# smoggy-P/gym-Drone2D-ActivePerception

Measured on AMD Instinct MI355X. Metric: env-steps/sec (batched) at 10 agents, map_id=1, higher is better.
Workload: dtype f64

## Files before the change

gym-drone2d-activeperception_amd/csrc/d2d_plugins.h:

```cpp

#define D2D_SINCOS_QUAL __device__ __forceinline__
#define D2D_SINCOS_TBL_QUAL __device__ const
#include "d2d_sincos.h"
#define D2D_ATAN2_QUAL __device__ __forceinline__
#define D2D_ATAN2_TBL_QUAL __device__ const
#include "d2d_atan2.h"
#define D2D_POW2_QUAL __device__ __forceinline__
#define D2D_POW2_TBL_QUAL __device__ const
#include "d2d_pow2.h"

__device__ __forceinline__ double norm2(double x, double y) { return sqrt(__builtin_fma(y, y, x * x)); }

__device__ __forceinline__ double shfl_f64(double v, int src) {
  int lo = __double2loint(v), hi = __double2hiint(v);
  lo = __shfl(lo, src, WAVE);
  hi = __shfl(hi, src, WAVE);
  return __hiloint2double(hi, lo);
}

template <int N>
__device__ __forceinline__ double row_shl_f64(double v) {
  int lo = __double2loint(v), hi = __double2hiint(v);
  lo = __builtin_amdgcn_update_dpp(lo, lo, 0x100 + N, 0xf, 0xf, false);
  hi = __builtin_amdgcn_update_dpp(hi, hi, 0x100 + N, 0xf, 0xf, false);
  return __hiloint2double(hi, lo);
}

template <int N>
__device__ __forceinline__ int row_shr_i32(int v) { return __builtin_amdgcn_update_dpp(v, v, 0x110 + N, 0xf, 0xf, false); }
template <int N>
__device__ __forceinline__ double row_shr_f64(double v) {
  return __hiloint2double(row_shr_i32<N>(__double2hiint(v)), row_shr_i32<N>(__double2loint(v)));
}
__device__ __forceinline__ double readlane_f64(double v, int l) {
  return __hiloint2double(__builtin_amdgcn_readlane(__double2hiint(v), l), __builtin_amdgcn_readlane(__double2loint(v), l));
}

__device__ __forceinline__ int wave_argmin(double t, int idx) {
  double m = t;
  m = __builtin_fmin(m, row_shr_f64<1>(m));
  m = __builtin_fmin(m, row_shr_f64<2>(m));
  m = __builtin_fmin(m, row_shr_f64<4>(m));
  m = __builtin_fmin(m, row_shr_f64<8>(m));
  const double wmin = __builtin_fmin(__builtin_fmin(readlane_f64(m, 15), readlane_f64(m, 31)),
                                     __builtin_fmin(readlane_f64(m, 47), readlane_f64(m, 63)));
  const unsigned long long eq = __ballot(t == wmin);
  if (__popcll(eq) == 1) return __builtin_amdgcn_readlane(idx, __ffsll((long long)eq) - 1);
  int c = (t == wmin) ? idx : 0x7fffffff;
  c = min(c, row_shr_i32<1>(c));
  c = min(c, row_shr_i32<2>(c));
  c = min(c, row_shr_i32<4>(c));
  c = min(c, row_shr_i32<8>(c));
  return min(min(__builtin_amdgcn_readlane(c, 15), __builtin_amdgcn_readlane(c, 31)),
             min(__builtin_amdgcn_readlane(c, 47), __builtin_amdgcn_readlane(c, 63)));
}

__device__ __forceinline__ double wave_fmin(double m) {
  m = __builtin_fmin(m, row_shr_f64<1>(m));
  m = __builtin_fmin(m, row_shr_f64<2>(m));
  m = __builtin_fmin(m, row_shr_f64<4>(m));
  m = __builtin_fmin(m, row_shr_f64<8>(m));
  return __builtin_fmin(__builtin_fmin(readlane_f64(m, 15), readlane_f64(m, 31)), __builtin_fmin(readlane_f64(m, 47), readlane_f64(m, 63)));
}
__device__ __forceinline__ double wave_fmax(double m) {
  m = __builtin_fmax(m, row_shr_f64<1>(m));
  m = __builtin_fmax(m, row_shr_f64<2>(m));
  m = __builtin_fmax(m, row_shr_f64<4>(m));
  m = __builtin_fmax(m, row_shr_f64<8>(m));
  return __builtin_fmax(__builtin_fmax(readlane_f64(m, 15), readlane_f64(m, 31)), __builtin_fmax(readlane_f64(m, 47), readlane_f64(m, 63)));
}

struct TrkView {
  double *mx, *my, *vx, *vy;
  double *lim;
  int n;
};

__device__ __forceinline__ double sq_threshold(double L) {
  if (!(L >= 0.0)) return -1.0;
  double t = L * L;
  for (int k = 0; k < 8 && sqrt(t) > L; ++k) t = __longlong_as_double(__double_as_longlong(t) - 1);
  for (int k = 0; k < 8; ++k) {
    const double u = __longlong_as_double(__double_as_longlong(t) + 1);
    if (!(sqrt(u) <= L)) break;
    t = u;
  }
  return t;
}

template <int WIDTH>
__device__ __forceinline__ bool plan_hits_round(const TrkView &T, int q, double x, double y, double t) {
  double mx[WIDTH], my[WIDTH], vx[WIDTH], vy[WIDTH], lim[WIDTH];
#pragma unroll
  for (int u = 0; u < WIDTH; ++u) {
    mx[u] = T.mx[q + u]; my[u] = T.my[q + u]; vx[u] = T.vx[q + u]; vy[u] = T.vy[q + u]; lim[u] = T.lim[q + u];
  }
  bool hit = false;
#pragma unroll
  for (int u = 0; u < WIDTH; ++u) {
    const double ex = mx[u] + t * vx[u], ey = my[u] + t * vy[u];
    const double dx = x - ex, dy = y - ey;
    hit = hit | ((q + u < T.n) & (__builtin_fma(dy, dy, dx * dx) <= lim[u]));
  }
  return hit;
}

__device__ __forceinline__ bool plan_hits_tracker(const TrkView &T, double x, double y, double t) {
  if (T.n <= 2) return T.n > 0 ? plan_hits_round<2>(T, 0, x, y, t) : false;
  bool hit = false;
  for (int q = 0; q < T.n; q += 4) hit = hit | plan_hits_round<4>(T, q, x, y, t);
  return hit;
}

template <typename DM>
__device__ __forceinline__ bool plan_is_free(const d2d_cfg &c, const d2d_plan &p, DM dm,
                                             const TrkView &T, double x, double y, double t, double inv_scale) {
  if (x != x || y != y) return false;
  const double d = p.safe_dist;
  const double xl = x - d, xr = x + d, yl = y - d, yr = y + d;
  const int W1 = c.W - 1, H1 = c.H - 1;
  const int i0 = min(max(cell_fast(xl, c.scale, inv_scale), 0), W1), i1 = min(max(cell_fast(x, c.scale, inv_scale), 0), W1),
            i2 = min(max(cell_fast(xr, c.scale, inv_scale), 0), W1);
  const int j0 = min(max(cell_fast(yl, c.scale, inv_scale), 0), H1), j1 = min(max(cell_fast(y, c.scale, inv_scale), 0), H1),
            j2 = min(max(cell_fast(yr, c.scale, inv_scale), 0), H1);
  const unsigned char v0 = dm[grid_ix(c, i0, j1)], v1 = dm[grid_ix(c, i1, j1)], v2 = dm[grid_ix(c, i2, j1)], v3 = dm[grid_ix(c, i1, j0)],
                      v4 = dm[grid_ix(c, i1, j2)];
  const bool ox0 = (xl >= c.W_px) | (xl < 0.0), ox1 = (x >= c.W_px) | (x < 0.0), ox2 = (xr >= c.W_px) | (xr < 0.0);
  const bool oy0 = (yl >= c.H_px) | (yl < 0.0), oy1 = (y >= c.H_px) | (y < 0.0), oy2 = (yr >= c.H_px) | (yr < 0.0);
  const bool wall = (ox0 | oy1 | (v0 == D2D_OCCUPIED)) | (ox1 | oy1 | (v1 == D2D_OCCUPIED)) | (ox2 | oy1 | (v2 == D2D_OCCUPIED)) |
                    (ox1 | oy0 | (v3 == D2D_OCCUPIED)) | (ox1 | oy2 | (v4 == D2D_OCCUPIED));
  return !wall && !plan_hits_tracker(T, x, y, t);
}

template <typename DM>
__device__ __forceinline__ bool plan_wall_int(const d2d_cfg &c, DM dm, int xi, int yi, int di, int Wpx, int Hpx) {
  const int xl = xi - di, xr = xi + di, yl = yi - di, yr = yi + di;
  const bool ox0 = (unsigned int)xl >= (unsigned int)Wpx, ox1 = (unsigned int)xi >= (unsigned int)Wpx, ox2 = (unsigned int)xr >= (unsigned int)Wpx;
  const bool oy0 = (unsigned int)yl >= (unsigned int)Hpx, oy1 = (unsigned int)yi >= (unsigned int)Hpx, oy2 = (unsigned int)yr >= (unsigned int)Hpx;
  const int Wm = Wpx - 1, Hm = Hpx - 1;
#define D2D_BY10(v, m) ((int)(__umul24((unsigned int)min(max((v), 0), (m)), 52429u) >> 19))
  const int W1 = c.W - 1, H1 = c.H - 1;
  const int i0 = min(D2D_BY10(xl, Wm), W1), i1 = min(D2D_BY10(xi, Wm), W1), i2 = min(D2D_BY10(xr, Wm), W1);
  const int j0 = min(D2D_BY10(yl, Hm), H1), j1 = min(D2D_BY10(yi, Hm), H1), j2 = min(D2D_BY10(yr, Hm), H1);
#undef D2D_BY10
  const unsigned char v0 = dm[grid_ix(c, i0, j1)], v1 = dm[grid_ix(c, i1, j1)], v2 = dm[grid_ix(c, i2, j1)], v3 = dm[grid_ix(c, i1, j0)],
                      v4 = dm[grid_ix(c, i1, j2)];
  return (ox0 | oy1 | (v0 == D2D_OCCUPIED)) | (ox1 | oy1 | (v1 == D2D_OCCUPIED)) | (ox2 | oy1 | (v2 == D2D_OCCUPIED)) |
         (ox1 | oy0 | (v3 == D2D_OCCUPIED)) | (ox1 | oy2 | (v4 == D2D_OCCUPIED));
}


__device__ __forceinline__ long long node_key(double px, double py, double vx, double vy) {
  const int a = cell_fast(rint(px), 10.0, 0.1), b = cell_fast(rint(py), 10.0, 0.1);
  const int cc = (int)rint(vx), d = (int)rint(vy);
  const unsigned int hi = ((unsigned int)(a + 32768) << 16) | ((unsigned int)(b + 32768) & 0xffffu);
  const unsigned int lo = ((unsigned int)(cc + 32768) << 16) | ((unsigned int)(d + 32768) & 0xffffu);
  return (long long)(((unsigned long long)hi << 32) | lo);
}

__device__ __forceinline__ unsigned int key_hash(long long k) {
  return (unsigned int)(((unsigned long long)k * 0x9E3779B97F4A7C15ull) >> 32);
}

#define NR_POS 0
#define NR_VEL 2
#define NR_COST 4
#define NR_META 6
#define NR_ACC 8
struct NodeRecs {
  double *b;
  __device__ __forceinline__ double *rec(int i) const { return b + (size_t)i * D2D_NODE_F; }
};
__device__ __forceinline__ double2 ld2(const double *q) { return *(const double2 *)q; }
__device__ __forceinline__ void st2(double *q, double a, double b) { *(double2 *)q = make_double2(a, b); }
__device__ __forceinline__ double meta_pack(int parent, int itr, int state) { return __hiloint2double((itr << 2) | state, parent); }
__device__ __forceinline__ int meta_parent(double m) { return __double2loint(m); }
__device__ __forceinline__ int meta_itr(double m) { return __double2hiint(m) >> 2; }
__device__ __forceinline__ int meta_state(double m) { return __double2hiint(m) & 3; }

#ifndef D2D_TRAJ_PRUNE_CHUNKS
#define D2D_TRAJ_PRUNE_CHUNKS 4
#endif
__device__ __forceinline__ double *traj_boxes(const d2d_plan &p, int e) {
  return p.traj_box ? (double *)p.traj_box + (size_t)e * ((p.traj_cap + WAVE - 1) / WAVE) * 4 : nullptr;
}

#define LH_N 1024
#define LH_MAX 896

#ifdef D2D_SEARCH_PROF
__device__ unsigned long long d2d_search_prof[16];
#define SP_T(var)                                              \
  do {                                                         \
    asm volatile("s_waitcnt vmcnt(0) lgkmcnt(0)" ::: "memory"); \
    var = __builtin_amdgcn_s_memtime();                        \
  } while (0)
#define SP_ADD(idx, t0, t1) \
  do {                      \
    spacc[idx] += (t1) - (t0); \
  } while (0)
#define SP_FLUSH()                                                            \
  do {                                                                        \
    if (e == 0 && lane == 0)                                                  \
      for (int spi = 0; spi < 16; ++spi) d2d_search_prof[spi] += spacc[spi]; \
  } while (0)
#else
#define SP_T(var) do { } while (0)
#define SP_ADD(idx, t0, t1) do { } while (0)
#define SP_FLUSH() do { } while (0)
#endif

struct SearchLds {
  int *chain;
  double *us;
  double *st;
  double *pc;
  double *rv;
  long long *rk;
  int *ri;
  int *misc;
  double *tot;
  int ntot;
  unsigned long long *prow;
  unsigned short *lh;
};

__host__ __device__ inline int search_lds_nodes(int N) { return N > 64 ? 256 : 512; }
__host__ __device__ inline bool search_wall_rows(int W, int H) { return W <= 64 && H <= 64; }

__device__ int plan_search(const d2d_cfg &c, const d2d_state &s, const d2d_plan &p, int e, int lane, const TrkView &T,
                           const SearchLds &S, const unsigned char *__restrict__ dm, double inv_scale) {
  const double H = p.horizon;
  const NodeRecs nd = {p.nodes + (size_t)e * p.node_cap * D2D_NODE_F};
  int *__restrict__ tab = p.hash + (size_t)e * p.hash_cap;
  double *__restrict__ traj = p.traj + (size_t)e * p.traj_cap * 4;
  int *stat = p.plan_stat + (size_t)e * 4;
  int *chain = S.chain;
  const unsigned int hmask = (unsigned int)p.hash_cap - 1u;
  const double tx = s.target[(size_t)e * 2], ty = s.target[(size_t)e * 2 + 1];
  const double *dr = s.drone + (size_t)e * D2D_DF;

  unsigned long long spa = 0, spb = 0;
  (void)spa; (void)spb;
#ifdef D2D_SEARCH_PROF
  unsigned long long spacc[16] = {0, 0, 0, 0, 0, 0, 0, 0, 0, 0, 0, 0, 0, 0, 0, 0};
#endif
  SP_T(spa);
  for (int i = lane; i < p.nu; i += WAVE) S.us[i] = p.u_space[i];
  {
    const FastDiv fdu(p.nu);
    for (int i = lane; i < p.nu * p.nu; i += WAVE) {
      int ia, ja;
      fdu.divmod(i, ia, ja);
      const double ax = p.u_space[ia], ay = p.u_space[ja];
      S.pc[i] = (ax * ax + ay * ay) / 100;
    }
  }
  for (int i = lane; i < 2 * p.n_sample; i += WAVE) S.st[i] = p.sample_t[i];
  {
    uint4 *lh128 = (uint4 *)S.lh;
    for (int i = lane; i < LH_N / 8; i += WAVE) lh128[i] = make_uint4(0u, 0u, 0u, 0u);
  }
  const bool int_walls = c.scale == 10.0 && c.W_px <= 81919.0 && c.H_px <= 81919.0 && c.W_px == floor(c.W_px) &&
                         c.H_px == floor(c.H_px) && c.W_px >= 1.0 && c.H_px >= 1.0 && p.safe_dist >= 0.0 &&
                         p.safe_dist <= 1048576.0 && p.safe_dist == floor(p.safe_dist);
  const int safe_i = int_walls ? (int)p.safe_dist : 0, wpx_i = int_walls ? (int)c.W_px : 1, hpx_i = int_walls ? (int)c.H_px : 1;
  const int kcell = safe_i / 10;
  const bool rows = S.prow != nullptr && int_walls && c.W <= 64 && c.H <= 64 && c.W_px == 10.0 * (double)c.W &&
                    c.H_px == 10.0 * (double)c.H && safe_i == 10 * kcell && 2 * kcell <= min(c.W, c.H);
  if (rows) {
    int olo = 0, ohi = 0;
    unsigned long long *orow = (unsigned long long *)S.rk;
    const int nb = c.W * c.H;
    if (c.grid_tile == 0 && (nb & 3) == 0 && (((size_t)dm) & 3) == 0) {
      orow[lane] = 0ull;
      const unsigned int *src = (const unsigned int *)dm;
      const FastDiv fdh(c.H);
      for (int d0 = 0; d0 < nb / 4; d0 += 10 * WAVE) {
        unsigned int x[10];
#pragma unroll
        for (int u = 0; u < 10; ++u) {
          const int idx = d0 + u * WAVE + lane;
          x[u] = src[min(idx, nb / 4 - 1)];
        }
#pragma unroll
        for (int u = 0; u < 10; ++u) {
          const int idx = d0 + u * WAVE + lane;
          const unsigned int y = x[u] ^ 0x01010101u;
          unsigned int z = ~(((y & 0x7f7f7f7fu) + 0x7f7f7f7fu) | y | 0x7f7f7f7fu);
          if (idx >= nb / 4) z = 0u;
          while (z) {
            const int b = (__ffs((int)z) - 1) >> 3;
            z &= z - 1u;
            int i, j;
            fdh.divmod_big(4 * idx + b, i, j);
            atomicOr(&orow[i], 1ull << j);
          }
        }
      }
      wave_sync_lds();
      const unsigned long long o = orow[lane];
      olo = (int)(unsigned int)o;
      ohi = (int)(unsigned int)(o >> 32);
      wave_sync_lds();
    } else {
      const int jc = min(lane, c.H - 1);
      for (int i0 = 0; i0 < c.W; i0 += 8) {
        unsigned char v[8];
#pragma unroll
        for (int u = 0; u < 8; ++u) v[u] = dm[grid_ix(c, min(i0 + u, c.W - 1), jc)];
#pragma unroll
        for (int u = 0; u < 8; ++u) {
          if (i0 + u < c.W) {
            const unsigned long long m = __ballot(lane < c.H && v[u] == D2D_OCCUPIED);
            olo = lane == i0 + u ? (int)(unsigned int)m : olo;
            ohi = lane == i0 + u ? (int)(unsigned int)(m >> 32) : ohi;
          }
        }
      }
    }
    const unsigned long long occ = ((unsigned long long)(unsigned int)ohi << 32) | (unsigned int)olo;
    orow[lane] = occ;
    wave_sync_lds();
    const unsigned long long up = orow[max(lane - kcell, 0)], dn = orow[min(lane + kcell, WAVE - 1)];
    const unsigned long long edge = kcell > 0 ? ((1ull << kcell) - 1ull) : 0ull;
    const unsigned long long edge_hi = kcell > 0 ? (edge << (c.H - kcell)) : 0ull;
    unsigned long long pr = occ | up | dn | (occ << kcell) | (occ >> kcell) | edge | edge_hi;
    if (lane < kcell || lane >= c.W - kcell) pr = ~0ull;
    wave_sync_lds();
    S.prow[lane] = pr;
  }
  const double kInf = __longlong_as_double(0x7ff0000000000000ll);
  const double vmax2 = p.vmax_sq != 0.0 ? p.vmax_sq : (p.vmax > 0.0 ? sq_threshold(__longlong_as_double(__double_as_longlong(p.vmax) - 1)) : -1.0);
  const double goal2 = p.goal_sq != 0.0 ? p.goal_sq : sq_threshold(p.goal_tol);
  wave_sync_lds();
  if (lane == 0) {
    const double x = dr[D2D_D_X], y = dr[D2D_D_Y], vx = dr[D2D_D_VX], vy = dr[D2D_D_VY];
    const double tot0 = 0.0 + 0.5 * norm2(x - tx, y - ty) + 0.1 * norm2(vx, vy);
    const long long k = node_key(x, y, vx, vy);
    double *r0 = nd.rec(0);
    st2(r0 + NR_POS, x, y);
    st2(r0 + NR_VEL, vx, vy);
    st2(r0 + NR_COST, 0.0, __longlong_as_double(k));
    st2(r0 + NR_META, meta_pack(-1, 0, 1), tot0);
    st2(r0 + NR_ACC, 0.0, 0.0);
    const unsigned int h32 = key_hash(k);
    S.lh[h32 >> 22] = (unsigned short)((((h32 >> 17) & 0x1fu) << 11) | 1u);
    S.tot[0] = tot0;
  }
  wave_sync_global();
  SP_T(spb);
  SP_ADD(10, spa, spb);
  bool nodup;
  double amax = 0.0;
  {
    double dmin = 1e300;
    for (int i = lane; i < p.nu; i += WAVE) {
      const double ui = S.us[i];
      if (i + 1 < p.nu) dmin = fmin(dmin, S.us[i + 1] - ui);
      amax = fmax(amax, fabs(ui));
    }
    dmin = wave_fmin(dmin);
    amax = wave_fmax(amax);
    nodup = H * dmin > 1.0 + 1e-6;
  }
  int nn = 1, open_n = 1, goal = -1, itr = 0, expansions = 0;
  bool overflow = false;
  bool lds_dict = true;
  const int nprim = p.nu * p.nu;
  const unsigned long long lt_mask = (1ull << lane) - 1ull;
  const FastDiv fd_nu(p.nu), fd_ns(p.n_sample);
  const double reach_a = 0.5 * H * H * amax + 2.0;
  const bool ns_pow2 = (p.n_sample & (p.n_sample - 1)) == 0 && p.n_sample <= WAVE;
  const bool one_batch = false;
  double ax1 = 0.0, ay1 = 0.0;
  if (one_batch) {
    int ia, ja;
    fd_nu.divmod(lane < nprim ? lane : 0, ia, ja);
    ax1 = S.us[ia];
    ay1 = S.us[ja];
  }
  for (;;) {
    itr += 1;
    if (open_n == 0 || itr >= p.max_itr) break;
    unsigned long long sp0 = 0, sp1 = 0, sp2 = 0, sp3 = 0, sp4 = 0, sp5 = 0, sp6 = 0, sp7 = 0, sp8 = 0;
    (void)sp0; (void)sp1; (void)sp2; (void)sp3; (void)sp4; (void)sp5; (void)sp6; (void)sp7; (void)sp8;
    SP_T(sp0);
    double best = kInf;
    int bidx = 0x7fffffff;
    bool fenced = false;
    {
      const int nl = min(nn, S.ntot);
      for (int s0 = 0; s0 < nl; s0 += 4 * WAVE) {
        double t4[4];
#pragma unroll
        for (int u = 0; u < 4; ++u) t4[u] = S.tot[min(s0 + u * WAVE + lane, S.ntot - 1)];
#pragma unroll
        for (int u = 0; u < 4; ++u) {
          const int si = s0 + u * WAVE + lane;
          const bool take = (si < nl) & (t4[u] < best);
          best = take ? t4[u] : best;
          bidx = take ? si : bidx;
        }
      }
      if (nn > nl) {
        wave_sync_global();
        fenced = true;
      }
      for (int s0 = nl; s0 < nn; s0 += WAVE) {
        const int si = s0 + lane;
        const double2 mt = ld2(nd.rec(min(si, nn - 1)) + NR_META);
        const bool take = (si < nn) & (meta_state(mt.x) == 1) & (mt.y < best);
        best = take ? mt.y : best;
        bidx = take ? si : bidx;
      }
    }
    bidx = wave_argmin(best, bidx);
    if (!fenced) wave_sync_global();
    if (__builtin_amdgcn_readfirstlane(bidx) == 0x7fffffff) {
      int fb = 0x7fffffff;
      for (int s0 = 0; s0 < nn; s0 += WAVE) {
        const int si = s0 + lane;
        if (si < nn && fb == 0x7fffffff && meta_state(nd.rec(si)[NR_META]) == 1) fb = si;
      }
      for (int o = 32; o > 0; o >>= 1) fb = min(fb, __shfl_xor(fb, o, WAVE));
      bidx = fb;
    }
    const int cur = __builtin_amdgcn_readfirstlane(bidx);
    SP_T(sp1);
    SP_ADD(0, sp0, sp1);
    const double *rc = nd.rec(cur);
    const double2 cpos = ld2(rc + NR_POS), cvel = ld2(rc + NR_VEL);
    const double ccost = rc[NR_COST];
    const int citr = meta_itr(rc[NR_META]);
    const double px = cpos.x, py = cpos.y, vx = cvel.x, vy = cvel.y;
    const bool fits_all = int_walls && (fabs(px) + H * fabs(vx) + reach_a <= 4194304.0) && (fabs(py) + H * fabs(vy) + reach_a <= 4194304.0);
    SP_T(sp2);
    SP_ADD(1, sp1, sp2);
    if (__builtin_fma(py - ty, py - ty, (px - tx) * (px - tx)) <= goal2) {
      goal = cur;
      break;
    }
    if (lane == 0) {
      ((int *)(nd.rec(cur) + NR_META))[1] = (citr << 2) | 2;
      if (cur < S.ntot) S.tot[cur] = kInf;
    }
    open_n -= 1;
    expansions += 1;
    for (int p0 = 0; p0 < nprim && !overflow; p0 += WAVE) {
      const int pi = p0 + lane;
      bool ok = pi < nprim;
      double ax, ay;
      if (one_batch) {
        ax = ax1;
        ay = ay1;
      } else {
        int ia, ja;
        fd_nu.divmod(ok ? pi : 0, ia, ja);
        ax = S.us[ia];
        ay = S.us[ja];
      }
      const double hx = ax / 2, hy = ay / 2;
      const double vex = vx + (2 * H) * hx, vey = vy + (2 * H) * hy;
      ok = ok && (__builtin_fma(vey, vey, vex * vex) <= vmax2);
      const unsigned long long vm = __ballot(ok);
      const int myrank = __popcll(vm & lt_mask);
      SP_T(sp3);
      SP_ADD(2, sp2, sp3);
      {
        const int nv = __popcll(vm);
        double *rax = S.rv, *ray = (double *)S.rk;
        if (ok) {
          rax[myrank] = hx;
          ray[myrank] = hy;
        }
        wave_sync_lds();
        const int npair = nv * p.n_sample;
        const int my_lo = myrank * p.n_sample;
        int nfree = 0;
        for (int q0 = 0; q0 < npair; q0 += 2 * WAVE) {
          int pr[2], si[2];
          bool in[2], fr[2];
          double sxv[2], syv[2], tgv[2];
#pragma unroll
          for (int u = 0; u < 2; ++u) {
            const int q = q0 + u * WAVE + lane;
            in[u] = q < npair;
            fd_ns.divmod(in[u] ? q : 0, pr[u], si[u]);
          }
          double shx[2], shy[2], tt[2], tt2[2];
#pragma unroll
          for (int u = 0; u < 2; ++u) {
            shx[u] = rax[pr[u]]; shy[u] = ray[pr[u]]; tt[u] = S.st[2 * si[u]]; tt2[u] = S.st[2 * si[u] + 1];
          }
#pragma unroll
          for (int u = 0; u < 2; ++u) {
            const double sx = rint(__builtin_fma(tt2[u], shx[u], px + tt[u] * vx)), sy = rint(__builtin_fma(tt2[u], shy[u], py + tt[u] * vy));
            const double tg = tt[u] + (double)citr * H;
            sxv[u] = sx; syv[u] = sy; tgv[u] = tg;
          }
          if (fits_all) {
            bool wall[2];
#pragma unroll
            for (int u = 0; u < 2; ++u) {
              const int xi = (int)sxv[u], yi = (int)syv[u];
              if (rows) {
                const bool inside = ((unsigned int)xi < (unsigned int)wpx_i) & ((unsigned int)yi < (unsigned int)hpx_i);
                unsigned int ci = __umul24((unsigned int)xi, 52429u) >> 19;
                ci = ci < 63u ? ci : 63u;
                const unsigned int cj = (__umul24((unsigned int)yi, 52429u) >> 19) & 63u;
                wall[u] = !inside | (((S.prow[ci] >> cj) & 1ull) != 0ull);
              } else {
                wall[u] = plan_wall_int(c, dm, xi, yi, safe_i, wpx_i, hpx_i);
              }
            }
#pragma unroll
            for (int u = 0; u < 2; ++u) fr[u] = !wall[u] & !plan_hits_tracker(T, sxv[u], syv[u], tgv[u]);
          } else {
#pragma unroll
            for (int u = 0; u < 2; ++u) fr[u] = plan_is_free(c, p, dm, T, sxv[u], syv[u], tgv[u], inv_scale);
          }
#pragma unroll
          for (int u = 0; u < 2; ++u) {
            const unsigned long long fm = __ballot(in[u] & fr[u]);
            const int qb = q0 + u * WAVE;
            if (ns_pow2) {
              const unsigned int sh = (unsigned int)(my_lo - qb);
              if (sh < (unsigned int)WAVE) nfree = __popcll(p.n_sample >= WAVE ? fm : ((fm >> sh) & ((1ull << p.n_sample) - 1ull)));
            } else {
              const int lo = max(my_lo, qb) - qb, hi = min(my_lo + p.n_sample, qb + WAVE) - qb;
              if (hi > lo) {
                const unsigned long long w = fm >> lo;
                nfree += __popcll(hi - lo >= WAVE ? w : (w & ((1ull << (hi - lo)) - 1ull)));
              }
            }
          }
        }
        if (ok) ok = nfree == p.n_sample;
      }
      SP_T(sp4);
      SP_ADD(3, sp3, sp4);
      const double ex = rint((px + H * vx) + (H * H) * hx), ey = rint((py + H * vy) + (H * H) * hy);
      const double cost = ccost + S.pc[ok ? pi : 0] + 10;
      const long long key = node_key(ex, ey, vex, vey);
      const unsigned int h32 = key_hash(key);
      int slot = -1;
      int slot_state = 0;
      double slot_cost = 0.0;
      unsigned int h = 0;
      if (lds_dict) {
        h = h32 >> 22;
        const unsigned int fp = (h32 >> 17) & 0x1fu;
        if (ok) {
          for (int guard = 0; guard < LH_N; ++guard) {
            const unsigned int ent = S.lh[h];
            if (ent == 0u) break;
            if ((ent >> 11) == fp) {
              const int sl = (int)(ent & 0x7ffu) - 1;
              const double *r2 = nd.rec(sl);
              const double2 ck = ld2(r2 + NR_COST);
              const double m2 = r2[NR_META];
              if (__double_as_longlong(ck.y) == key) {
                slot = sl;
                slot_state = meta_state(m2);
                slot_cost = ck.x;
                break;
              }
            }
            h = (h + 1u) & (LH_N - 1u);
          }
        }
      } else {
        h = h32 & hmask;
        if (ok) {
          for (int guard = 0; guard < p.hash_cap; ++guard) {
            const int sv = __hip_atomic_load(&tab[h], __ATOMIC_RELAXED, __HIP_MEMORY_SCOPE_AGENT);
            if (sv == 0) break;
            const double *r2 = nd.rec(sv - 1);
            const double2 ck = ld2(r2 + NR_COST);
            const double m2 = r2[NR_META];
            if (__double_as_longlong(ck.y) == key) {
              slot = sv - 1;
              slot_state = meta_state(m2);
              slot_cost = ck.x;
              break;
            }
            h = (h + 1) & hmask;
          }
        }
      }
      SP_T(sp5);
      SP_ADD(4, sp4, sp5);
      const unsigned long long m = __ballot(ok);
      const int nok = __popcll(m), rank = __popcll(m & lt_mask);
      unsigned long long dupm = 0;
      if (!nodup) {
        unsigned long long *bk = (unsigned long long *)chain;
        bk[lane] = 0ull;
        const unsigned long long ukey = (unsigned long long)key;
        unsigned int hb = ((unsigned int)ukey + (unsigned int)(ukey >> 32) * 0x9E3779B1u) >> 26;
        const bool odd = ok & (ukey == 0ull);
        bool rep = false, pending = ok & !odd;
        for (int trip = 0; trip < WAVE && __any(pending); ++trip) {
          unsigned long long old = 0ull;
          if (pending) old = atomicCAS(&bk[hb], 0ull, ukey);
          const bool same = pending & (old == ukey);
          rep = rep | same;
          pending = pending & (old != 0ull) & !same;
          hb = (hb + 1u) & 63u;
        }
        dupm = __ballot(rep | odd);
      }
      int leader = lane, wlane = lane;
      double wcost = cost;
      if (dupm != 0ull) {
        wave_sync_lds();
        if (ok) {
          S.rk[rank] = key;
          S.rv[rank] = cost;
          S.ri[rank] = lane;
        }
        wave_sync_lds();
        leader = lane;
        wlane = -1;
        wcost = 0.0;
#pragma unroll 1
        for (int j = 0; j < nok; ++j) {
          const bool same = ok & (S.rk[j] == key);
          const int lj = S.ri[j];
          const double cj = S.rv[j];
          leader = (same & (lj < leader)) ? lj : leader;
          const bool better = same & ((wlane < 0) | (cj < wcost));
          wcost = better ? cj : wcost;
          wlane = better ? lj : wlane;
        }
      }
      if (!nodup) wave_sync_lds();
      SP_T(sp6);
      SP_ADD(5, sp5, sp6);
      const bool is_leader = ok && leader == lane;
      const bool exists = slot >= 0;
      const bool closed = exists & (slot_state == 2);
      const double ecost = slot_cost;
      const unsigned long long newm = __ballot(is_leader && !exists);
      const int nnew = __popcll(newm);
      if (nn + nnew > p.node_cap) {
        overflow = true;
        break;
      }
      int myslot = slot;
      if (is_leader && !exists) myslot = nn + __popcll(newm & lt_mask);
      const int gslot = dupm != 0ull ? __shfl(myslot, leader, WAVE) : myslot;
      const bool write = ok && wlane == lane && (!exists || (!closed && ecost > wcost));
      if (write) {
        double *rw = nd.rec(gslot);
        const double tot = cost + 0.5 * norm2(ex - tx, ey - ty) + 0.1 * norm2(vex, vey);
        st2(rw + NR_POS, ex, ey);
        st2(rw + NR_VEL, vex, vey);
        st2(rw + NR_COST, cost, __longlong_as_double(key));
        st2(rw + NR_META, meta_pack(cur, citr + 1, 1), tot);
        st2(rw + NR_ACC, ax, ay);
        if (gslot < S.ntot) S.tot[gslot] = tot;
      }
      if (lds_dict && (nn + nnew > LH_MAX)) {
        for (int i = lane; i < p.hash_cap; i += WAVE) tab[i] = 0;
        wave_sync_global();
        for (int s0 = 0; s0 < nn; s0 += WAVE) {
          const int si = s0 + lane;
          if (si < nn) {
            const long long k2 = __double_as_longlong(nd.rec(si)[NR_COST + 1]);
            unsigned int hh = key_hash(k2) & hmask;
            for (int guard = 0; guard < p.hash_cap; ++guard) {
              if (atomicCAS(&tab[hh], 0, si + 1) == 0) break;
              hh = (hh + 1) & hmask;
            }
          }
        }
        wave_sync_global();
        lds_dict = false;
        h = h32 & hmask;
      }
      if (is_leader && !exists) {
        if (lds_dict) {
          const unsigned int ent = (((h32 >> 17) & 0x1fu) << 11) | (unsigned int)(myslot + 1);
          unsigned int *lh32 = (unsigned int *)S.lh;
          for (int guard = 0; guard < 4 * LH_N; ++guard) {
            const unsigned int sh = (h & 1u) * 16u;
            const unsigned int w = lh32[h >> 1];
            if (((w >> sh) & 0xffffu) != 0u) {
              h = (h + 1u) & (LH_N - 1u);
              continue;
            }
            if (atomicCAS(&lh32[h >> 1], w, w | (ent << sh)) == w) break;
          }
        } else {
          unsigned int hh = h;
          for (int guard = 0; guard < p.hash_cap; ++guard) {
            if (atomicCAS(&tab[hh], 0, myslot + 1) == 0) break;
            hh = (hh + 1) & hmask;
          }
        }
      }
      nn += nnew;
      open_n += nnew;
      SP_T(sp7);
      SP_ADD(6, sp6, sp7);
      if (p0 + WAVE < nprim) wave_sync_global();
      else wave_sync_lds();
      SP_T(sp8);
      SP_ADD(7, sp7, sp8);
      SP_ADD(8, sp0, sp8);
#ifdef D2D_SEARCH_PROF
      spacc[9] += 1;
#endif
    }
    if (overflow) break;
  }
  if (lane == 0) {
    stat[0] += 1;
    stat[1] = expansions;
    stat[2] = nn;
    if (overflow) stat[3] = 1;
  }
  if (goal < 0 || overflow) {
    SP_FLUSH();
    return -1;
  }
  SP_T(spa);
  int depth = 0;
  for (int q = goal; q != 0 && depth <= 128; q = meta_parent(nd.rec(q)[NR_META])) depth += 1;
  if (depth * p.n_ts > p.traj_cap || depth > 128) {
    if (lane == 0) stat[3] = 1;
    return -1;
  }
  if (lane == 0) {
    int q = goal;
    for (int lvl = depth - 1; lvl >= 0; --lvl) {
      chain[lvl] = q;
      q = meta_parent(nd.rec(q)[NR_META]);
    }
  }
  wave_sync_lds();
  const int total = depth * p.n_ts;
  double *tbox = traj_boxes(p, e);
  for (int w0 = 0; w0 < total; w0 += WAVE) {
    const int w = w0 + lane;
    double ox = 0.0, oy = 0.0;
    if (w < total) {
      const int lvl = w / p.n_ts, mi = w - lvl * p.n_ts;
      const int q = chain[lvl];
      const double *rq = nd.rec(q);
      const int par = meta_parent(rq[NR_META]);
      const double2 acc = ld2(rq + NR_ACC);
      const double hx = acc.x / 2, hy = acc.y / 2;
      const double t = p.traj_t[3 * mi], t2 = p.traj_t[3 * mi + 1], tt = p.traj_t[3 * mi + 2];
      const double2 pp = ld2(nd.rec(par) + NR_POS), pv = ld2(nd.rec(par) + NR_VEL);
      double *o = traj + (size_t)w * 4;
      ox = rint(__builtin_fma(t2, hx, pp.x + t * pv.x));
      oy = rint(__builtin_fma(t2, hy, pp.y + t * pv.y));
      o[0] = ox;
      o[1] = oy;
      o[2] = pv.x + tt * hx;
      o[3] = pv.y + tt * hy;
    }
    if (tbox) {
      const bool on = w < total;
      const double xlo = wave_fmin(on ? ox : 1e300), ylo = wave_fmin(on ? oy : 1e300);
      const double xhi = wave_fmax(on ? ox : -1e300), yhi = wave_fmax(on ? oy : -1e300);
      if (lane == 0) {
        st2(tbox + 4 * (w0 / WAVE), xlo, ylo);
        st2(tbox + 4 * (w0 / WAVE) + 2, xhi, yhi);
      }
    }
  }
  SP_T(spb);
  SP_ADD(11, spa, spb);
#ifdef D2D_SEARCH_PROF
  spacc[12] += 1;
#endif
  SP_FLUSH();
  return total;
}

__host__ __device__ inline int plan_wave_bytes(int N, int nu, int n_sample, int W, int H) {
  const int ncap = ((N > 0 ? N : 1) + 3) & ~3;
  const int nu4 = ((nu + 3) & ~3) + ((nu * nu + 3) & ~3), ns4 = (2 * n_sample + 3) & ~3;
  const int rowb = search_wall_rows(W, H) ? 8 * 64 : 0;
  return 5 * 8 * ncap + 8 * (nu4 + ns4) + 8 * 64 + 8 * 64 + 4 * 64 + 128 * 4 + 16 + 8 * search_lds_nodes(N) + rowb + 2 * LH_N;
}

__device__ __forceinline__ void plan_carve(const d2d_cfg &c, const d2d_plan &p, char *base, TrkView &T, SearchLds &S) {
  const int N = c.N, ncap = ((N > 0 ? N : 1) + 3) & ~3;
  T.mx = (double *)base;
  T.my = T.mx + ncap;
  T.vx = T.my + ncap;
  T.vy = T.vx + ncap;
  T.lim = T.vy + ncap;
  S.us = T.lim + ncap;
  S.pc = S.us + ((p.nu + 3) & ~3);
  S.st = S.pc + ((p.nu * p.nu + 3) & ~3);
  S.rv = S.st + ((2 * p.n_sample + 3) & ~3);
  S.rk = (long long *)(S.rv + 64);
  S.ri = (int *)(S.rk + 64);
  S.chain = S.ri + 64;
  S.misc = S.chain + 128;
  S.tot = (double *)(S.misc + 4);
  S.ntot = search_lds_nodes(N);
  unsigned long long *after = (unsigned long long *)(S.tot + S.ntot);
  S.prow = search_wall_rows(c.W, c.H) ? after : nullptr;
  S.lh = (unsigned short *)(after + (search_wall_rows(c.W, c.H) ? 64 : 0));
}

__device__ __forceinline__ void plan_emit(const d2d_state &s, const d2d_plan &p, int e, int lane, int head, int stored, int ok,
                                          const double4 *w_head = nullptr) {
  if (lane == 0) {
    const double *traj = p.traj + (size_t)e * p.traj_cap * 4;
    int *hdr = p.traj_hdr + (size_t)e * 2;
    unsigned char *plan_ok = (unsigned char *)s.plan_ok, *wp_valid = (unsigned char *)s.wp_valid;
    double *wp = (double *)s.wp + (size_t)e * 6;
    plan_ok[e] = (unsigned char)ok;
    if (stored - head > 0) {
      double2 wa, wb;
      if (w_head) {
        wa = make_double2(w_head->x, w_head->y);
        wb = make_double2(w_head->z, w_head->w);
      } else {
        const double *w = traj + (size_t)head * 4;
        wa = ld2(w);
        wb = ld2(w + 2);
      }
      wp[0] = wa.x; wp[1] = wa.y; wp[2] = wb.x; wp[3] = wb.y; wp[4] = 0.0; wp[5] = 0.0;
      wp_valid[e] = 1;
      head += 1;
    } else {
      wp_valid[e] = 0;
      for (int i = 0; i < 6; ++i) wp[i] = 0.0;
    }
    hdr[0] = head;
    hdr[1] = stored;
  }
}

__device__ __forceinline__ bool plan_env_quick(const d2d_cfg &c, const d2d_state &s, const d2d_plan &p, int e, int lane, char *base,
                                               double4 *w_head_out = nullptr, int *walls_ok = nullptr) {
  const int N = c.N;
  TrkView T;
  SearchLds S;
  plan_carve(c, p, base, T, S);
  const double inv_scale = 1.0 / c.scale;
  const unsigned char *__restrict__ dm = s.dmap + (size_t)e * grid_bytes(c);
  int *hdr = p.traj_hdr + (size_t)e * 2;
  const int hdr_l = hdr[lane & 1];
  int nact = 0;
  for (int k0 = 0; k0 < N; k0 += WAVE) {
    const int k = k0 + lane;
    bool act = false;
    double m0 = 0, m1 = 0, m2 = 0, m3 = 0, rad = 0, lim2 = 0;
    if (k < N) {
      const double *mu = s.kf + ((size_t)e * N + k) * D2D_KF;
      m0 = mu[0]; m1 = mu[1]; m2 = mu[2]; m3 = mu[3];
      act = s.active[(size_t)e * N + k] != 0;
      const bool prev = p.trk_prev[(size_t)e * N + k] != 0;
      rad = p.trk_radius[(size_t)e * N + k];
      const double lim_in = p.trk_lim[(size_t)e * N + k];
      lim2 = lim_in;
      if (prev && !act) {
        rad = p.agent_radius;
        p.trk_radius[(size_t)e * N + k] = rad;
        lim2 = 0.0;
      }
      if (act && !(lim2 > 0.0)) lim2 = sq_threshold(c.drone_radius + rad);
      if (lim2 != lim_in) p.trk_lim[(size_t)e * N + k] = lim2;
      if (prev != act) p.trk_prev[(size_t)e * N + k] = act ? 1 : 0;
    }
    const unsigned long long am = __ballot(act);
    if (act) {
      const int q = nact + __popcll(am & ((1ull << lane) - 1ull));
      T.mx[q] = m0; T.my[q] = m1; T.vx[q] = m2; T.vy[q] = m3;
      T.lim[q] = lim2;
    }
    nact += __popcll(am);
  }
  T.n = nact;
  wave_sync_lds();
  int head = __builtin_amdgcn_readlane(hdr_l, 0), stored = __builtin_amdgcn_readlane(hdr_l, 1);
  double *__restrict__ traj = p.traj + (size_t)e * p.traj_cap * 4;
  double4 w_first = make_double4(0.0, 0.0, 0.0, 0.0);
  {
    const int n = stored - head;
    bool bad = false;
    const int c_lo = head >> 6, c_hi = n > 0 ? (stored - 1) >> 6 : c_lo - 1;
    const double *tbox = traj_boxes(p, e);
    const bool chunked = tbox != nullptr && c_hi - c_lo < 64 && c_hi - c_lo >= D2D_TRAJ_PRUNE_CHUNKS;
    const bool walls_known = walls_ok != nullptr && *walls_ok != 0 && n < 2560;
    unsigned long long cmask = 0ull;
    bool walls_full = true;
    if (__builtin_expect(chunked && n > 0, 0)) {
      const double2 dpos = ld2(s.drone + (size_t)e * D2D_DF);
      bool need = false;
      if (c_lo + lane <= c_hi) {
        const int cc = c_lo + lane;
        const double2 lo = ld2(tbox + 4 * cc), hi = ld2(tbox + 4 * cc + 2);
        need = cc == c_lo;
        if (!walls_known) {
          need = true;
        } else {
          const int reach = (int)((c.depth + 1.5 * (c.scale - 1.0)) / c.scale) + 2;
          const int ocx = cell_fast(dpos.x, c.scale, inv_scale), ocy = cell_fast(dpos.y, c.scale, inv_scale);
          const double wx0 = (double)(ocx - reach) * c.scale, wx1 = (double)(ocx + reach + 1) * c.scale;
          const double wy0 = (double)(ocy - reach) * c.scale, wy1 = (double)(ocy + reach + 1) * c.scale;
          need = need | ((hi.x >= wx0) & (lo.x < wx1) & (hi.y >= wy0) & (lo.y < wy1));
        }
        const int a_lo = max(cc << 6, head), a_hi = min((cc << 6) + 63, stored - 1);
        const double t_lo = (double)(a_lo - head) * c.dt, t_hi = (double)(a_hi - head) * c.dt;
        for (int q = 0; q < nact; ++q) {
          const double mxq = T.mx[q], myq = T.my[q], vxq = T.vx[q], vyq = T.vy[q];
          const double ex0 = mxq + t_lo * vxq, ex1 = mxq + t_hi * vxq, ey0 = myq + t_lo * vyq, ey1 = myq + t_hi * vyq;
          const double rad = sqrt(T.lim[q]) * (1.0 + 1e-9) + 1e-9;
          const double exl = fmin(ex0, ex1), exh = fmax(ex0, ex1), eyl = fmin(ey0, ey1), eyh = fmax(ey0, ey1);
          need = need | ((hi.x + rad >= exl) & (lo.x - rad <= exh) & (hi.y + rad >= eyl) & (lo.y - rad <= eyh));
        }
      }
      cmask = __ballot(need);
      walls_full = !walls_known;
    }
    auto visit = [&](int a, bool first) {
      if (a >= head && a < stored) {
        const int i = a - head;
        const double *w = traj + (size_t)a * 4;
        const double2 wxy = ld2(w), wv = ld2(w + 2);
        const double4 w4 = make_double4(wxy.x, wxy.y, wv.x, wv.y);
        if (first) w_first = w4;
        const double wx = w4.x, wy = w4.y;
        const double ti = (double)i * c.dt;
        const int ci = cell_fast(wx, c.scale, inv_scale), cj = cell_fast(wy, c.scale, inv_scale);
        const bool in = ci >= 0 && ci < c.W && cj >= 0 && cj < c.H;
        const int sv = ((int)ti) & 0xff;
        if (in && sv > 0 && dm[grid_ix(c, min(max(ci, 0), c.W - 1), min(max(cj, 0), c.H - 1))] == D2D_OCCUPIED) bad = true;
        for (int q = 0; q < nact; q += 4) {
          double mx[4], my[4], vx[4], vy[4], lim[4];
#pragma unroll
          for (int u = 0; u < 4; ++u) {
            mx[u] = T.mx[q + u]; my[u] = T.my[q + u]; vx[u] = T.vx[q + u]; vy[u] = T.vy[q + u]; lim[u] = T.lim[q + u];
          }
#pragma unroll
          for (int u = 0; u < 4; ++u) {
            const double ex = mx[u] + ti * vx[u], ey = my[u] + ti * vy[u];
            const double dx = ex - wx, dy = ey - wy;
            bad = bad | ((q + u < nact) & (__builtin_fma(dy, dy, dx * dx) <= lim[u]));
          }
        }
      }
    };
    if (__builtin_expect(chunked, 0)) {
      for (unsigned long long m = cmask; m; m &= m - 1ull) {
        const int cc = c_lo + __ffsll((long long)m) - 1;
// ... 986 lines not shown
```

Baseline: 89.28 million.

## Probe node dictionary before collision sampling and skip non-improving successors

Moves the hash-dictionary lookup ahead of the per-sample collision check. Successors that already exist closed, or that do not improve on an existing cost, are filtered out before the costly trajectory sampling, and the wave skips the rest of the iteration when no candidates remain. Adds a single-round path for when the sample pairs fit in one wave, and recomputes the primitive values afterwards to reduce register pressure. Moving the dominance check before collision and dedup could change which lane wins among duplicates relative to existing nodes, which risks subtle behaviour differences.

```diff
diff --git a/gym-drone2d-activeperception_amd/csrc/d2d_plugins.h b/gym-drone2d-activeperception_amd/csrc/d2d_plugins.h
--- a/gym-drone2d-activeperception_amd/csrc/d2d_plugins.h
+++ b/gym-drone2d-activeperception_amd/csrc/d2d_plugins.h
@@ -210,6 +210,11 @@
 #define SP_FLUSH() do { } while (0)
 #endif
 
+template <int N>
+struct IntC {
+  static constexpr int value = N;
+};
+
 struct SearchLds {
   int *chain;
   double *us;
@@ -460,87 +465,12 @@
         ax = S.us[ia];
         ay = S.us[ja];
       }
-      const double hx = ax / 2, hy = ay / 2;
-      const double vex = vx + (2 * H) * hx, vey = vy + (2 * H) * hy;
+      double hx = ax / 2, hy = ay / 2;
+      double vex = vx + (2 * H) * hx, vey = vy + (2 * H) * hy;
       ok = ok && (__builtin_fma(vey, vey, vex * vex) <= vmax2);
-      const unsigned long long vm = __ballot(ok);
-      const int myrank = __popcll(vm & lt_mask);
       SP_T(sp3);
       SP_ADD(2, sp2, sp3);
-      {
-        const int nv = __popcll(vm);
-        double *rax = S.rv, *ray = (double *)S.rk;
-        if (ok) {
-          rax[myrank] = hx;
-          ray[myrank] = hy;
-        }
-        wave_sync_lds();
-        const int npair = nv * p.n_sample;
-        const int my_lo = myrank * p.n_sample;
-        int nfree = 0;
-        for (int q0 = 0; q0 < npair; q0 += 2 * WAVE) {
-          int pr[2], si[2];
-          bool in[2], fr[2];
-          double sxv[2], syv[2], tgv[2];
-#pragma unroll
-          for (int u = 0; u < 2; ++u) {
-            const int q = q0 + u * WAVE + lane;
-            in[u] = q < npair;
-            fd_ns.divmod(in[u] ? q : 0, pr[u], si[u]);
-          }
-          double shx[2], shy[2], tt[2], tt2[2];
-#pragma unroll
-          for (int u = 0; u < 2; ++u) {
-            shx[u] = rax[pr[u]]; shy[u] = ray[pr[u]]; tt[u] = S.st[2 * si[u]]; tt2[u] = S.st[2 * si[u] + 1];
-          }
-#pragma unroll
-          for (int u = 0; u < 2; ++u) {
-            const double sx = rint(__builtin_fma(tt2[u], shx[u], px + tt[u] * vx)), sy = rint(__builtin_fma(tt2[u], shy[u], py + tt[u] * vy));
-            const double tg = tt[u] + (double)citr * H;
-            sxv[u] = sx; syv[u] = sy; tgv[u] = tg;
-          }
-          if (fits_all) {
-            bool wall[2];
-#pragma unroll
-            for (int u = 0; u < 2; ++u) {
-              const int xi = (int)sxv[u], yi = (int)syv[u];
-              if (rows) {
-                const bool inside = ((unsigned int)xi < (unsigned int)wpx_i) & ((unsigned int)yi < (unsigned int)hpx_i);
-                unsigned int ci = __umul24((unsigned int)xi, 52429u) >> 19;
-                ci = ci < 63u ? ci : 63u;
-                const unsigned int cj = (__umul24((unsigned int)yi, 52429u) >> 19) & 63u;
-                wall[u] = !inside | (((S.prow[ci] >> cj) & 1ull) != 0ull);
-              } else {
-                wall[u] = plan_wall_int(c, dm, xi, yi, safe_i, wpx_i, hpx_i);
-              }
-            }
-#pragma unroll
-            for (int u = 0; u < 2; ++u) fr[u] = !wall[u] & !plan_hits_tracker(T, sxv[u], syv[u], tgv[u]);
-          } else {
-#pragma unroll
-            for (int u = 0; u < 2; ++u) fr[u] = plan_is_free(c, p, dm, T, sxv[u], syv[u], tgv[u], inv_scale);
-          }
-#pragma unroll
-          for (int u = 0; u < 2; ++u) {
-            const unsigned long long fm = __ballot(in[u] & fr[u]);
-            const int qb = q0 + u * WAVE;
-            if (ns_pow2) {
-              const unsigned int sh = (unsigned int)(my_lo - qb);
-              if (sh < (unsigned int)WAVE) nfree = __popcll(p.n_sample >= WAVE ? fm : ((fm >> sh) & ((1ull << p.n_sample) - 1ull)));
-            } else {
-              const int lo = max(my_lo, qb) - qb, hi = min(my_lo + p.n_sample, qb + WAVE) - qb;
-              if (hi > lo) {
-                const unsigned long long w = fm >> lo;
-                nfree += __popcll(hi - lo >= WAVE ? w : (w & ((1ull << (hi - lo)) - 1ull)));
-              }
-            }
-          }
-        }
-        if (ok) ok = nfree == p.n_sample;
-      }
-      SP_T(sp4);
-      SP_ADD(3, sp3, sp4);
-      const double ex = rint((px + H * vx) + (H * H) * hx), ey = rint((py + H * vy) + (H * H) * hy);
+      double ex = rint((px + H * vx) + (H * H) * hx), ey = rint((py + H * vy) + (H * H) * hy);
       const double cost = ccost + S.pc[ok ? pi : 0] + 10;
       const long long key = node_key(ex, ey, vex, vey);
       const unsigned int h32 = key_hash(key);
@@ -589,9 +519,121 @@
           }
         }
       }
+      const bool exists = slot >= 0;
+      ok = ok && (!exists || ((slot_state != 2) & (slot_cost > cost)));
+      const unsigned long long vm = __ballot(ok);
+      SP_T(sp4);
+      SP_ADD(3, sp3, sp4);
+      if (vm == 0ull) {
+        wave_sync_lds();
+#ifdef D2D_SEARCH_PROF
+        spacc[9] += 1;
+        spacc[13] += 1;
+        SP_T(sp8);
+        SP_ADD(8, sp0, sp8);
+#endif
+        continue;
+      }
+      const int myrank = __popcll(vm & lt_mask);
+      {
+        const int nv = __popcll(vm);
+        double *rax = S.rv, *ray = (double *)S.rk;
+        if (ok) {
+          rax[myrank] = hx;
+          ray[myrank] = hy;
+        }
+        wave_sync_lds();
+        const int npair = nv * p.n_sample;
+        const int my_lo = myrank * p.n_sample;
+        int nfree = 0;
+        auto pair_rounds = [&](auto nr_c, const int q0) __attribute__((always_inline)) {
+          constexpr int NR = decltype(nr_c)::value;
+          int pr[NR], si[NR];
+          bool in[NR], fr[NR];
+          double sxv[NR], syv[NR], tgv[NR];
+#pragma unroll
+          for (int u = 0; u < NR; ++u) {
+            const int q = q0 + u * WAVE + lane;
+            in[u] = q < npair;
+            fd_ns.divmod(in[u] ? q : 0, pr[u], si[u]);
+          }
+          double shx[NR], shy[NR], tt[NR], tt2[NR];
+#pragma unroll
+          for (int u = 0; u < NR; ++u) {
+            shx[u] = rax[pr[u]]; shy[u] = ray[pr[u]]; tt[u] = S.st[2 * si[u]]; tt2[u] = S.st[2 * si[u] + 1];
+          }
+#pragma unroll
+          for (int u = 0; u < NR; ++u) {
+            const double sx = rint(__builtin_fma(tt2[u], shx[u], px + tt[u] * vx)), sy = rint(__builtin_fma(tt2[u], shy[u], py + tt[u] * vy));
+            const double tg = tt[u] + (double)citr * H;
+            sxv[u] = sx; syv[u] = sy; tgv[u] = tg;
+          }
+          if (fits_all) {
+            bool wall[NR];
+#pragma unroll
+            for (int u = 0; u < NR; ++u) {
+              const int xi = (int)sxv[u], yi = (int)syv[u];
+              if (rows) {
+                const bool inside = ((unsigned int)xi < (unsigned int)wpx_i) & ((unsigned int)yi < (unsigned int)hpx_i);
+                unsigned int ci = __umul24((unsigned int)xi, 52429u) >> 19;
+                ci = ci < 63u ? ci : 63u;
+                const unsigned int cj = (__umul24((unsigned int)yi, 52429u) >> 19) & 63u;
+                wall[u] = !inside | (((S.prow[ci] >> cj) & 1ull) != 0ull);
+              } else {
+                wall[u] = plan_wall_int(c, dm, xi, yi, safe_i, wpx_i, hpx_i);
+              }
+            }
+#pragma unroll
+            for (int u = 0; u < NR; ++u) fr[u] = !wall[u] & !plan_hits_tracker(T, sxv[u], syv[u], tgv[u]);
+          } else {
+#pragma unroll
+            for (int u = 0; u < NR; ++u) fr[u] = plan_is_free(c, p, dm, T, sxv[u], syv[u], tgv[u], inv_scale);
+          }
+#pragma unroll
+          for (int u = 0; u < NR; ++u) {
+            const unsigned long long fm = __ballot(in[u] & fr[u]);
+            const int qb = q0 + u * WAVE;
+            if (ns_pow2) {
+              const unsigned int sh = (unsigned int)(my_lo - qb);
+              if (sh < (unsigned int)WAVE) nfree = __popcll(p.n_sample >= WAVE ? fm : ((fm >> sh) & ((1ull << p.n_sample) - 1ull)));
+            } else {
+              const int lo = max(my_lo, qb) - qb, hi = min(my_lo + p.n_sample, qb + WAVE) - qb;
+              if (hi > lo) {
+                const unsigned long long w = fm >> lo;
+                nfree += __popcll(hi - lo >= WAVE ? w : (w & ((1ull << (hi - lo)) - 1ull)));
+              }
+            }
+          }
+        };
+        if (npair <= WAVE) {
+          pair_rounds(IntC<1>{}, 0);
+#ifdef D2D_SEARCH_PROF
+          spacc[14] += 1;
+#endif
+        } else {
+          for (int q0 = 0; q0 < npair; q0 += 2 * WAVE) pair_rounds(IntC<2>{}, q0);
+        }
+        if (ok) ok = nfree == p.n_sample;
+      }
       SP_T(sp5);
       SP_ADD(4, sp4, sp5);
+      asm volatile("" : "+v"(ax), "+v"(ay));
+      hx = ax / 2;
+      hy = ay / 2;
+      vex = vx + (2 * H) * hx;
+      vey = vy + (2 * H) * hy;
+      ex = rint((px + H * vx) + (H * H) * hx);
+      ey = rint((py + H * vy) + (H * H) * hy);
       const unsigned long long m = __ballot(ok);
+      if (m == 0ull) {
+        wave_sync_lds();
+#ifdef D2D_SEARCH_PROF
+        spacc[9] += 1;
+        SP_T(sp8);
+        SP_ADD(8, sp0, sp8);
+#endif
+        continue;
+      }
       const int nok = __popcll(m), rank = __popcll(m & lt_mask);
       unsigned long long dupm = 0;
       if (!nodup) {
@@ -639,9 +681,6 @@
       SP_T(sp6);
       SP_ADD(5, sp5, sp6);
       const bool is_leader = ok && leader == lane;
-      const bool exists = slot >= 0;
-      const bool closed = exists & (slot_state == 2);
-      const double ecost = slot_cost;
       const unsigned long long newm = __ballot(is_leader && !exists);
       const int nnew = __popcll(newm);
       if (nn + nnew > p.node_cap) {
@@ -651,7 +690,7 @@
       int myslot = slot;
       if (is_leader && !exists) myslot = nn + __popcll(newm & lt_mask);
       const int gslot = dupm != 0ull ? __shfl(myslot, leader, WAVE) : myslot;
-      const bool write = ok && wlane == lane && (!exists || (!closed && ecost > wcost));
+      const bool write = ok && wlane == lane;
       if (write) {
         double *rw = nd.rec(gslot);
         const double tot = cost + 0.5 * norm2(ex - tx, ey - ty) + 0.1 * norm2(vex, vey);
```

After: 91.19 million, median of 6. 1.02x the previous value.
